# OSU-Bee-Lab/buzzdetect

Measured on AMD Instinct MI355X. Metric: yamnet_windows_per_s, higher is better.
Workload: dtype f32 (split-f16x3 MFMA products, f32 accumulate)

## Files before the change

buzzdetect_amd/csrc/bd_device.h:

```cpp
#pragma once

#include "bd_internal.h"

#include <mutex>
#include <type_traits>
#ifdef BD_KERNEL_TRACE
#include <cstdio>
#include <cstdlib>
#endif

namespace bd {

namespace {

typedef float f32x16 __attribute__((ext_vector_type(16)));
typedef float v2f __attribute__((ext_vector_type(2)));
typedef float v4f __attribute__((ext_vector_type(4)));
typedef unsigned v4u __attribute__((ext_vector_type(4)));
typedef unsigned u32x2 __attribute__((ext_vector_type(2)));
typedef _Float16 f16x2 __attribute__((ext_vector_type(2)));
typedef _Float16 f16x4 __attribute__((ext_vector_type(4)));
typedef _Float16 f16x8 __attribute__((ext_vector_type(8)));

constexpr float kF16Max = 65504.0f;
// ... 70 lines not shown
                                    }
                    }
    return true;
}
static_assert(tr_image_is_bijection(), "every (half, k, chunk) has its own 8 bytes of the slot, and they fill it");
static_assert(tr_image_writes_conflict_free(), "a lane group of the publication meets no bank twice");
static_assert(tr_image_reads_conflict_free(), "a lane half of the transposed read meets no bank twice");
__device__ __forceinline__ int tr_read_lane_off(int lane) {
    const int g = lane >> 4, q = (lane >> 2) & 3, p = lane & 3;
    return tr_image_off(0, tr_read_k(0, g >> 1, 0, q), tr_read_chunk(0, g & 1, p));
}
__host__ __device__ constexpr int tr_read_next(int off) { return (off ^ 16) + 4 * kTrRowBytes; }
constexpr bool tr_read_next_holds() {
    for (int lane = 0; lane < 64; ++lane) {
        const int g = lane >> 4, q = (lane >> 2) & 3, p = lane & 3;
        if (tr_read_next(tr_image_off(0, tr_read_k(0, g >> 1, 0, q), tr_read_chunk(0, g & 1, p))) !=
            tr_image_off(0, tr_read_k(0, g >> 1, 1, q), tr_read_chunk(0, g & 1, p)))
            return false;
        for (int s = 0; s < 2; ++s)
            for (int i = 0; i < 3; ++i)
                for (int r = 0; r < 2; ++r)
                    if (tr_image_off(0, tr_read_k(s, g >> 1, r, q), tr_read_chunk(i, g & 1, p)) !=
                        tr_image_off(0, tr_read_k(0, g >> 1, r, q), tr_read_chunk(0, g & 1, p)) + 16 * s * kTrRowBytes + 64 * i)
                        return false;
    }
    return true;
}
static_assert(tr_read_next_holds(), "the reader's immediates");
__device__ __forceinline__ f16x8 tr_read_frag(const char* p0, const char* p1) {
    typedef short s16x4 __attribute__((ext_vector_type(4)));
    typedef __attribute__((address_space(3))) s16x4* lds4;
    const s16x4 a = __builtin_amdgcn_ds_read_tr16_b64_v4i16((lds4)p0), b = __builtin_amdgcn_ds_read_tr16_b64_v4i16((lds4)p1);
    return __builtin_bit_cast(f16x8, __builtin_shufflevector(a, b, 0, 1, 2, 3, 4, 5, 6, 7));
}

__device__ __forceinline__ unsigned pw_lds_addr(const void* p) {
    return (unsigned)(unsigned long long)(__attribute__((address_space(3))) const void*)p;
}
template <int OFFSET>
__device__ __forceinline__ f16x8 pw_lds_frag(unsigned addr) {
    f16x8 v;
    asm volatile("ds_read_b128 %0, %1 offset:%2" : "=v"(v) : "v"(addr), "n"(OFFSET) : "memory");
    return v;
}
__device__ __forceinline__ void pw_lds_store64(unsigned addr, f16x4 v) {
    asm volatile("ds_write_b64 %0, %1" ::"v"(addr), "v"(v) : "memory");
}
__device__ __forceinline__ f16x8 pw_landed(f16x8 v) {
    asm volatile("" : "+v"(v));
    return v;
}
template <int N>
__device__ __forceinline__ void pw_lds_wait() {
    asm volatile("s_waitcnt lgkmcnt(%0)" ::"n"(N) : "memory");
}
template <int I, int E, typename F>
__device__ __forceinline__ void static_for_pw(F&& f) {
    if constexpr (I < E) {
        f(std::integral_constant<int, I>{});
        static_for_pw<I + 1, E>(f);
    }
}
template <int K16, int V, int R>
struct PwResSchedule {
    static constexpr int split_at(int q) {
        for (int j = 0; j < V; ++j)
// ... 60 lines not shown
```

buzzdetect_amd/csrc/bd_internal.h:

```cpp
#pragma once

#include <hip/hip_runtime.h>
#include <stdint.h>

#include <string>
#include <vector>

#include "../../include/buzzdetect_hip.h"

namespace bd {

constexpr int kMelNonZero = 461;

constexpr int kMelStart[BD_MEL_BANDS] = {
    5, 5, 6, 7, 9, 10, 11, 12, 13, 14, 16, 17, 18, 20, 21, 23, 25, 26, 28, 30, 32, 34, 36, 38, 40, 42, 44, 47, 49, 52, 54, 57,
    60, 63, 66, 69, 72, 76, 79, 83, 87, 90, 95, 99, 103, 108, 112, 117, 122, 127, 133, 138, 144, 150, 156, 162, 169, 176, 183,
    190, 198, 206, 214, 223};
constexpr int kMelLen[BD_MEL_BANDS] = {
    1, 2, 3, 3, 2, 2, 2, 2, 3, 3, 2, 3, 3, 3, 4, 3, 3, 4, 4, 4, 4, 4, 4, 4, 4, 5, 5, 5, 5, 5, 6, 6,
    6, 6, 6, 7, 7, 7, 8, 7, 8, 9, 8, 9, 9, 9, 10, 10, 11, 11, 11, 12, 12, 12, 13, 14, 14, 14, 15, 16, 16, 17, 17, 17};
constexpr int mel_offset(int band) {
    int o = 0;
    for (int m = 0; m < band; ++m) o += kMelLen[m];
    return o;
// ... 133 lines not shown
                  const SepLayer& L2, const SepLayer& L3, float* out, hipStream_t stream);

void launch_stem_reg(const float* logmel, int patch_step, const WindowMap& map, int w0, int windows, const float* c1_w,
                     const float* c1_b, const SepLayer& L2, const SepLayer& L3, float* out, hipStream_t stream);
void launch_stem_reg_planes(const float* logmel, int patch_step, const WindowMap& map, int w0, int windows, const float* c1_w,
                            const float* c1_b, const SepLayer& L2, const SepLayer& L3, float* out, hipStream_t stream);

void launch_stem_reg_f32(const float* logmel, int patch_step, const WindowMap& map, int w0, int windows, const float* c1_w,
                         const float* c1_b, const SepLayer& L2, const SepLayer& L3, float* out, hipStream_t stream);

bool launch_l4_reg_f32(const float* in, float* out, int windows, const SepLayer& L4, const SepLayer& L5, hipStream_t stream);

bool launch_separable_mid(const float* in, float* out, int windows, const SepLayer& L5, const SepLayer& L6, const SepLayer& L7,
                          hipStream_t stream);
constexpr int kDw7PlaneBytes = 8 * 2 * 24 * 32 * 2;
bool separable_mid_planes_supported(const SepLayer& L5, const SepLayer& L6, const SepLayer& L7);
bool launch_separable_mid_planes(const float* in, void* out, int windows, const SepLayer& L5, const SepLayer& L6, const SepLayer& L7,
                                 hipStream_t stream);

bool launch_separable_mid_f32(const float* in, float* out, int windows, const SepLayer& L5, const SepLayer& L6, const SepLayer& L7,
                              hipStream_t stream);

bool separable_chip_pw7_supported(const SepLayer& L7, const SepLayer* L, int nl, const SepLayer& next, int windows);
bool launch_separable_chip_pw7(const void* in, float* out, int windows, const SepLayer& L7, const SepLayer* L, int nl,
                               const SepLayer& next, hipStream_t stream);
int launch_separable_run_next_dw(const float* a, float* b, int windows, const SepLayer* L, int max_layers, hipStream_t stream,
                                 bool planes = false);

bool launch_separable_chip_f32(const float* in, float* out, int windows, const SepLayer* L, int nl, hipStream_t stream,
                               const SepLayer* next, bool dw0_done);

bool tail_supported(const SepLayer& L13, const SepLayer& L14);
bool launch_tail_pw13_dw14(const void* in, void* out, int windows, const SepLayer& L13, const SepLayer& L14, hipStream_t stream);
bool launch_tail_pw14_pool(const void* in, float* pooled, int windows, const SepLayer& L14, hipStream_t stream);
bool tail_f32_supported(const SepLayer& L13, const SepLayer& L14);
bool launch_tail_f32(const float* in, float* mid, float* pooled, int windows, const SepLayer& L13, const SepLayer& L14, hipStream_t stream,
                     int which);

struct DenseLayer {
    int k, n;
    int act;
    const float* wfrag;
    const float* bias;
};
size_t dense_packed_floats(int k, int n);
void dense_pack_weights(const float* kernel, int k, int n, float* dst);
void launch_dense(const float* A, int lda, int windows, const DenseLayer& L, float* C, int ldc, hipStream_t stream);
void launch_softmax_rows(const float* x, int ldx, float* y, int windows, int n, hipStream_t stream);

}

struct bd_headset_member;

namespace bd {

constexpr int kHeadSetRow = 2048;
constexpr int kHeadSetRegions = 3;
struct HeadSet {
    int members = 0, outputs = 0;
    std::vector<int> first, count;
    std::vector<int> last_act;
    char* dev = nullptr;
    struct Depth {
        const void* layers;
        const void* tiles;
        int n_tiles;
    };
// ... 33 lines not shown
```

buzzdetect_amd/csrc/cnn.hip:

```cpp
#include "bd_device.h"

namespace bd {

namespace {

constexpr int kC1Rows = 4;

__global__ __launch_bounds__(256) void conv1_kernel(const float* __restrict__ logmel, int patch_step,
                                                    const WindowMap map, int w0,
                                                    const float* __restrict__ w9x32,
                                                    const float* __restrict__ b32,
                                                    float* __restrict__ out) {
    const int tid = threadIdx.x;
    const int c4 = tid & 7;
    const int ow = tid >> 3;
    const int win = blockIdx.y;
    const float* patch = logmel + window_frame(map, w0 + win, patch_step) * BD_MEL_BANDS;

    float4 wt[9];
#pragma unroll
    for (int t = 0; t < 9; ++t) wt[t] = reinterpret_cast<const float4*>(w9x32 + t * 32)[c4];
    const float4 bias = reinterpret_cast<const float4*>(b32)[c4];

#pragma unroll
// ... 609 lines not shown
    __shared__ float s_part[4][BD_MAX_CLASSES];
    const int tid = threadIdx.x;
    const int lane = tid & 63;
    const int wave = tid >> 6;
    const size_t win = blockIdx.x;
    const float4* src = reinterpret_cast<const float4*>(act + win * POOL * BD_EMBEDDING_SIZE);
    float4 s = src[tid];
    if constexpr (POOL > 1) {
#pragma unroll
        for (int p = 1; p < POOL; ++p) {
            const float4 v = src[p * (BD_EMBEDDING_SIZE / 4) + tid];
            s.x += v.x;
            s.y += v.y;
            s.z += v.z;
            s.w += v.w;
        }
        s.x /= (float)POOL;
        s.y /= (float)POOL;
        s.z /= (float)POOL;
        s.w /= (float)POOL;
        if (emb) reinterpret_cast<float4*>(emb + win * BD_EMBEDDING_SIZE)[tid] = s;
    }
    if (!logits) return;

    for (int c0 = 0; c0 < n_classes; c0 += 16) {
        float4 w[16];
#pragma unroll
        for (int j = 0; j < 16; ++j) {
            const int c = c0 + j < n_classes ? c0 + j : n_classes - 1;
            w[j] = reinterpret_cast<const float4*>(head_wt + (size_t)c * BD_EMBEDDING_SIZE)[tid];
        }
        float p[16];
#pragma unroll
        for (int j = 0; j < 16; ++j) p[j] = fmaf(s.x, w[j].x, fmaf(s.y, w[j].y, fmaf(s.z, w[j].z, s.w * w[j].w)));
#pragma unroll
        for (int o = 32; o > 0; o >>= 1)
#pragma unroll
            for (int j = 0; j < 16; ++j) p[j] += __shfl_xor(p[j], o, 64);
#pragma unroll
        for (int j = 0; j < 16; ++j)
            if (lane == 0 && c0 + j < n_classes) s_part[wave][c0 + j] = p[j];
    }
    __syncthreads();
    if (tid < n_classes)
        logits[win * n_classes + tid] =
            ((s_part[0][tid] + s_part[1][tid]) + (s_part[2][tid] + s_part[3][tid])) + head_b[tid];
}

}

void launch_conv1(const float* logmel, int patch_step, const WindowMap& map, int w0, int windows, const float* w9x32,
                  const float* b32, float* out, hipStream_t stream) {
    if (windows <= 0) return;
    hipLaunchKernelGGL(conv1_kernel, dim3(48 / kC1Rows, windows), dim3(256), 0, stream, logmel, patch_step, map, w0,
                       w9x32, b32, out);
}

template <int STRIDE, int OWB>
static void launch_dw(const float* in, float* out, int windows, const SepLayer& L, hipStream_t stream) {
    const long long total = (long long)windows * L.h_out * (L.w_out / OWB) * (L.cin / 4);
    const long long blocks = (total + 255) / 256;
    const int grid = (int)(blocks < (1 << 20) ? blocks : (1 << 20));
    hipLaunchKernelGGL((depthwise_kernel<STRIDE, OWB>), dim3(grid), dim3(256), 0, stream, in, out, dw_w_of(L), dw_b_of(L),
                       windows, L.h_in, L.w_in, L.cin, L.h_out, L.w_out, L.amax);
}

void launch_scale_copy(const float* src, float* dst, int64_t n, float factor, hipStream_t stream) {
// ... 164 lines not shown
```

buzzdetect_amd/csrc/engine.hip:

```cpp
#include <cmath>
#include <cstdio>
#include <cstdlib>
#include <cstring>
#include <unistd.h>
#include <memory>
#include <string>
#include <type_traits>
#include <utility>
#include <vector>

#include "bd_internal.h"

#include "../../include/buzzdetect_anyrate.h"
#include "../../include/buzzdetect_head.h"
#include "../../include/buzzdetect_headset.h"
#include "../../include/buzzdetect_ensemble.h"

namespace {

thread_local std::string g_error;

int fail(int code, const std::string& msg) {
    g_error = msg;
    return code;
// ... 2 lines not shown
#define BD_HIP(expr)                                                                            \
    do {                                                                                        \
        hipError_t e_ = (expr);                                                                 \
        if (e_ != hipSuccess)                                                                   \
            return fail(BD_EHIP, std::string(#expr) + ": " + hipGetErrorString(e_));            \
    } while (0)

const int kLayerDefs[14][2] = {{2, 32},  {1, 64},  {2, 128}, {1, 128}, {2, 256}, {1, 256},  {2, 512},
                               {1, 512}, {1, 512}, {1, 512}, {1, 512}, {1, 512}, {2, 1024}, {1, 1024}};

constexpr int64_t kFloatsA = 98304;
constexpr int64_t kFloatsB = 49152;
constexpr int kDefaultGroup = 1024;
constexpr int kMaxGroup = 65536;
static_assert(kMaxGroup <= 1 << 17, "the tail launchers of pass_f16 / pass_f32 cover the largest pass");
static_assert(bd::kDw7PlaneBytes <= kFloatsA * 4, "the depthwise-7 planes of the middle run fit buffer a");

inline int64_t align_up(int64_t v, int64_t a) { return (v + a - 1) / a * a; }

struct Event2 {
    hipEvent_t ev;
    int slot;
};

}

struct bd_engine {
    int device = 0;
    int n_classes = 0;
    int group_windows = kDefaultGroup;
    int pointwise_mode = 1;
    unsigned* d_range_flag = nullptr;
    int stem = 3, separable = 1;
    float* d_pool = nullptr;
    bd::FeTables* d_tables = nullptr;
    std::vector<float> h_dw[13];
    std::vector<int> row_exp[13];
    size_t off_dw16[13] = {0}, off_pw_u[13] = {0};
    float act_max[13] = {0};
    int act_exp[13] = {0};
    unsigned* d_amax = nullptr;
    const float* conv1_w = nullptr;
    const float* conv1_b = nullptr;
    bd::SepLayer sep[13];
    const float* head_wt = nullptr;
    const float* head_b = nullptr;
    std::vector<bd::DenseLayer> stack;
    float* d_stack = nullptr;
    bd::HeadSet set;
    bd::Ensemble ens;
    struct Taps {
        int up, down, quality, half;
        float* dev;
        std::vector<float> host;
        bool has_plan;
        bd::FirPlanHost fir;
        hipStream_t upload_stream;
        hipEvent_t uploaded;
    };
    std::vector<Taps> taps;
    struct AnyTaps {
        bd::AnyratePlan plan;
        int quality;
        float* dev;
        std::vector<float> host;
        hipStream_t upload_stream;
// ... 345 lines not shown
            const int kq = cin / 16;
            for (int n = 0; n < cout; ++n)
                for (int k = 0; k < cin; ++k) {
                    const int lane = (n & 31) + 32 * ((k & 15) >> 3);
                    const size_t dst = (((size_t)(n >> 5) * kq + (k >> 4)) * 64 + lane) * 8 + (k & 7);
                    fhi[dst] = hi[(size_t)n * cin + k];
                    flo[dst] = lo[(size_t)n * cin + k];
                }
        }
        off_pw_ffrag[l] = 0;
        if (cin >= 128) {
            off_pw_ffrag[l] = reserve(nw);
            const float* wf = host.data() + off_pw_w[l];
            float* ff = host.data() + off_pw_ffrag[l];
            const int ks = cin / 8;
            for (int n = 0; n < cout; ++n)
                for (int k = 0; k < cin; ++k) {
                    const int lane = (n & 31) + 32 * ((k & 7) >> 2);
                    ff[(((size_t)(n >> 5) * ks + (k >> 3)) * 64 + lane) * 4 + (k & 3)] = wf[(size_t)n * cin + k];
                }
        }
        cin = cout;
    }
    if (p - w->embedder_blob != BD_EMBEDDER_BLOB_FLOATS) return fail(BD_EWEIGHTS, "internal: blob walk mismatch");
    size_t off_head_w = 0, off_head_b = 0;
    if (w->n_classes > 0) {
        off_head_w = reserve((size_t)w->n_classes * BD_EMBEDDING_SIZE);
        off_head_b = reserve(BD_MAX_CLASSES);
        for (int c = 0; c < w->n_classes; ++c)
            for (int k = 0; k < BD_EMBEDDING_SIZE; ++k)
                host[off_head_w + (size_t)c * BD_EMBEDDING_SIZE + k] = w->head_kernel[(size_t)k * w->n_classes + c];
        for (int c = 0; c < w->n_classes; ++c) host[off_head_b + c] = w->head_bias[c];
    }
    {
        bool finite = true;
        for (size_t i = off_conv1_w; i < off_conv1_b + 32; ++i) finite = finite && std::isfinite(host[i]);
        int c = kLayerDefs[0][1];
        for (int l = 0; l < 13; ++l) {
            const int co = kLayerDefs[l + 1][1];
            for (size_t i = 0; i < 9 * (size_t)c; ++i) finite = finite && std::isfinite(host[off_dw_w[l] + i]);
            for (int i = 0; i < c; ++i) finite = finite && std::isfinite(host[off_dw_b[l] + i]);
            for (size_t i = 0; i < (size_t)c * co; ++i) finite = finite && std::isfinite(host[off_pw_w[l] + i]);
            for (int i = 0; i < co; ++i) finite = finite && std::isfinite(host[off_pw_b[l] + i]);
            c = co;
        }
        if (!finite) return fail(BD_EWEIGHTS, "bd_create: non-finite value after BatchNorm folding");
    }

    bd::FeTables tables;
    int rc = build_tables(w->mel, &tables);
    if (rc < 0) return rc;

    bd_engine* e = new bd_engine();
    e->device = device;
    e->n_classes = w->n_classes;
    hipError_t err = hipMalloc(&e->d_pool, host.size() * sizeof(float));
    if (err == hipSuccess) err = hipMalloc(&e->d_tables, sizeof(bd::FeTables));
    if (err == hipSuccess) err = hipMalloc(&e->d_range_flag, 256);
    if (err == hipSuccess) err = hipMemset(e->d_range_flag, 0, 256);
    if (err == hipSuccess) err = hipMalloc(&e->d_amax, 64);
    if (err == hipSuccess) err = hipMemset(e->d_amax, 0, 64);
    if (err == hipSuccess) err = hipMemcpy(e->d_pool, host.data(), host.size() * sizeof(float), hipMemcpyHostToDevice);
    if (err == hipSuccess) err = hipMemcpy(e->d_tables, &tables, sizeof(tables), hipMemcpyHostToDevice);
    if (err != hipSuccess) {
        if (e->d_pool) (void)hipFree(e->d_pool);
        if (e->d_tables) (void)hipFree(e->d_tables);
        if (e->d_range_flag) (void)hipFree(e->d_range_flag);
        if (e->d_amax) (void)hipFree(e->d_amax);
        delete e;
        return fail(BD_EHIP, std::string("bd_create: ") + hipGetErrorString(err));
    }
    e->conv1_w = e->d_pool + off_conv1_w;
    e->conv1_b = e->d_pool + off_conv1_b;
    int h = 48, wd = 32;
    cin = kLayerDefs[0][1];
    for (int l = 0; l < 13; ++l) {
        bd::SepLayer& L = e->sep[l];
        L.cin = cin;
        L.cout = kLayerDefs[l + 1][1];
        L.stride = kLayerDefs[l + 1][0];
        L.h_in = h;
        L.w_in = wd;
        L.h_out = (h + L.stride - 1) / L.stride;
        L.w_out = (wd + L.stride - 1) / L.stride;
        L.dw_w = e->d_pool + off_dw_w[l];
        L.dw_b = e->d_pool + off_dw_b[l];
        L.pw_wt = e->d_pool + off_pw_w[l];
        L.pw_b = e->d_pool + off_pw_b[l];
        L.pw_variant = 0;
        L.pw_whi = e->d_pool + off_pw_hi[l];
        L.pw_wlo = e->d_pool + off_pw_lo[l];
        L.pw_fhi = e->d_pool + off_pw_fhi[l];
        L.pw_flo = e->d_pool + off_pw_flo[l];
        L.pw_ffrag = off_pw_ffrag[l] ? e->d_pool + off_pw_ffrag[l] : nullptr;
        L.pw_variant16 = 0;
        L.pw_mode = e->pointwise_mode;
        L.range_flag = e->d_range_flag;
        L.dw_w16 = e->d_pool + off_dw16[l];
        L.dw_b16 = L.dw_w16 + 9 * (size_t)cin;
        L.pw_u = e->d_pool + off_pw_u[l];
        L.act_exp = 0;
        L.amax = nullptr;
        e->off_dw16[l] = off_dw16[l];
        e->off_pw_u[l] = off_pw_u[l];
        e->row_exp[l] = row_exps[l];
// ... 450 lines not shown
        stem(g, bd::launch_stem_reg_planes);
        if (!g.launch(7, [&] { return bd::launch_l4_window_planes(g.a, sep[1], sep[2], sep[3], g.b, g.gw, g.stream); }))
            return fail(BD_EHIP, "l4_window_kernel declined the planes of the stem");
    } else {
        if (e->stem != 0) {
            stem(g, e->stem == 3 ? bd::launch_stem_reg : bd::launch_stem4);
        } else {
            conv1(g);
            walk_layers(g, 0, false, 4);
        }
        if (e->separable == 0) return walk_layers(g, 2, false, -1);
        if (!g.launch(7, [&] { return bd::launch_separable_fused_next_dw(g.a, g.b, g.gw, sep[2], sep[3], g.stream); }))
            return walk_layers(g, 2, false, -1);
    }
    const bool planes = bd::tail_supported(sep[11], sep[12]);
    if (e->separable == 1 && planes && bd::separable_mid_planes_supported(sep[3], sep[4], sep[5]) &&
        bd::separable_chip_pw7_supported(sep[5], &sep[6], 5, sep[11], g.gw)) {
        if (!g.launch(13, [&] { return bd::launch_separable_mid_planes(g.b, g.a, g.gw, sep[3], sep[4], sep[5], g.stream); }))
            return fail(BD_EHIP, "sep_mid_kernel declined the depthwise-7 planes");
        if (!g.launch(23, [&] { return bd::launch_separable_chip_pw7(g.a, g.b, g.gw, sep[5], &sep[6], 5, sep[11], g.stream); }))
            return fail(BD_EHIP, "sep_chip_kernel declined the planes of the middle run");
    } else {
        if (!(e->separable == 1 &&
              g.launch(13, [&] { return bd::launch_separable_mid(g.b, g.a, g.gw, sep[3], sep[4], sep[5], g.stream); }))) {
            pointwise(g, 3);
            if (!g.launch(11, [&] { return bd::launch_separable_fused_next_dw(g.a, g.b, g.gw, sep[4], sep[5], g.stream); }))
                return walk_layers(g, 4, false, -1);
            pointwise(g, 5);
        }
        if (!g.launch(23, [&] { return bd::launch_separable_run_next_dw(g.a, g.b, g.gw, &sep[6], 7, g.stream, planes); }))
            return walk_layers(g, 6, false, -1);
        if (!planes) return walk_layers(g, 11, true, -1);
    }
    float* const pooled = g.emb ? g.emb : g.b;
    if (!g.launch(25, [&] { return bd::launch_tail_pw13_dw14(g.b, g.a, g.gw, sep[11], sep[12], g.stream); }) ||
        !g.launch(27, [&] { return bd::launch_tail_pw14_pool(g.a, pooled, g.gw, sep[12], g.stream); }))
        return fail(BD_EHIP, "septail.hip declined the planes of the on-chip run");
    return head(g, pooled);
}

int pass_f32(Group& g) {
    const bd_engine* e = g.e;
    const bd::SepLayer* sep = g.sep;
    stem(g, bd::launch_stem_reg_f32);
    if (e->separable == 0) return walk_layers(g, 2, false, -1);
    if (!g.launch(7, [&] { return bd::launch_l4_reg_f32(g.a, g.b, g.gw, sep[2], sep[3], g.stream); }))
        return walk_layers(g, 2, false, -1);
    bool dw8_done = false;
    if (!(e->separable == 1 &&
          g.launch(13, [&] { return bd::launch_separable_mid_f32(g.b, g.a, g.gw, sep[3], sep[4], sep[5], g.stream); }))) {
        for (int l = 3; l < 6; ++l) {
            if (!g.launch(3 + 2 * l, [&] { return bd::launch_pointwise_next_dw_f32(g.b, g.a, g.gw, sep[l], sep[l + 1], g.stream); }))
                return walk_layers(g, l, true, -1);
            std::swap(g.a, g.b);
        }
        dw8_done = true;
    }
    if (!g.launch(23, [&] {
            return dw8_done ? bd::launch_separable_chip_f32(g.b, g.a, g.gw, &sep[6], 5, g.stream, &sep[11], true)
                            : bd::launch_separable_chip_f32(g.a, g.b, g.gw, &sep[6], 5, g.stream, &sep[11], false);
        }))
        return walk_layers(g, 6, dw8_done, -1);
    if (dw8_done) std::swap(g.a, g.b);
    if (!bd::tail_f32_supported(sep[11], sep[12])) return walk_layers(g, 11, true, -1);
    float* const pooled = g.emb ? g.emb : g.b;
    if (!g.launch(25, [&] { return bd::launch_tail_f32(g.b, g.a, pooled, g.gw, sep[11], sep[12], g.stream, 0); }) ||
        !g.launch(27, [&] { return bd::launch_tail_f32(g.b, g.a, pooled, g.gw, sep[11], sep[12], g.stream, 1); }))
        return fail(BD_EHIP, "septail.hip declined the exact-f32 tail");
    return head(g, pooled);
// ... 288 lines not shown
        if (act_exp[l] < -60 || act_exp[l] > 60) return fail(BD_EINVAL, "bd_set_activation_exponents: exponent outside -60..60");
    for (int l = 0; l < 13; ++l) h->act_exp[l] = act_exp[l];
    return apply_scales(h);
}

int bd_stage_tap(bd_handle h, const float* pcm_dev, int64_t n_samples, int32_t hop_samples, int32_t patch_step,
                 void* workspace_dev, int64_t workspace_bytes, int32_t stage, int32_t windows, float* out_dev,
                 void* stream) {
    if (!out_dev) return fail(BD_EINVAL, "bd_stage_tap: null output");
    if (stage < 0 || stage >= BD_NUM_STAGES) return fail(BD_EINVAL, "bd_stage_tap: stage out of range");
    return run_packed(h, pcm_dev, &n_samples, 1, hop_samples, patch_step, workspace_dev, workspace_bytes, nullptr,
                      nullptr, stage, windows, out_dev, (hipStream_t)stream);
}

int bd_debug_pointwise(const float* a_dev, const float* wt_dev, const float* bias_dev, float* c_dev, int64_t m,
                       int32_t n, int32_t k, int32_t variant, void* stream) {
    if (!a_dev || !wt_dev || !bias_dev || !c_dev || m < 0) return fail(BD_EINVAL, "bd_debug_pointwise: bad argument");
    if (bd::launch_pointwise_variant(a_dev, wt_dev, bias_dev, c_dev, m, n, k, variant, (hipStream_t)stream) != 0)
        return fail(BD_EINVAL, "bd_debug_pointwise: shape/variant not supported (K % 32, N % tile)");
    BD_HIP(hipGetLastError());
    return BD_OK;
}

int bd_set_pointwise_variant(bd_handle h, int32_t layer, int32_t variant) {
    if (!h || layer < 2 || layer > 14) return fail(BD_EINVAL, "bd_set_pointwise_variant: layer must be 2..14");
    if (h->sep[layer - 2].pw_mode != 0) h->sep[layer - 2].pw_variant16 = variant;
    else h->sep[layer - 2].pw_variant = variant;
    return BD_OK;
}

int bd_set_fusion(bd_handle h, int32_t stem, int32_t separable) {
    if (!h) return fail(BD_EINVAL, "null handle");
    if (stem != 0 && stem != 3 && stem != 5) return fail(BD_EINVAL, "bd_set_fusion: stem must be 0, 3 or 5");
    if (separable != 0 && separable != 1 && separable != 10)
        return fail(BD_EINVAL, "bd_set_fusion: separable must be 0, 1 or 10");
    h->stem = stem;
    h->separable = separable;
    return BD_OK;
}

int bd_range_flag(bd_handle h, int32_t* flag_host, int32_t reset, void* stream) {
    if (!h || !flag_host) return fail(BD_EINVAL, "bd_range_flag: null argument");
    BD_HIP(hipSetDevice(h->device));
    unsigned v = 0;
    BD_HIP(hipMemcpyAsync(&v, h->d_range_flag, sizeof(v), hipMemcpyDeviceToHost, (hipStream_t)stream));
    BD_HIP(hipStreamSynchronize((hipStream_t)stream));
    if (reset && v) BD_HIP(hipMemsetAsync(h->d_range_flag, 0, sizeof(v), (hipStream_t)stream));
    *flag_host = (int32_t)v;
    return BD_OK;
}

int bd_range_flag_copy(bd_handle h, int32_t* dst, int32_t reset, void* stream) {
    if (!h || !dst) return fail(BD_EINVAL, "bd_range_flag_copy: null argument");
    BD_HIP(hipSetDevice(h->device));
    BD_HIP(hipMemcpyAsync(dst, h->d_range_flag, sizeof(int32_t), hipMemcpyDefault, (hipStream_t)stream));
    if (reset) BD_HIP(hipMemsetAsync(h->d_range_flag, 0, sizeof(int32_t), (hipStream_t)stream));
    return BD_OK;
}

int bd_set_pointwise_mode(bd_handle h, int32_t mode) {
    if (!h || mode < 0 || mode > 2)
        return fail(BD_EINVAL, "bd_set_pointwise_mode: mode must be 0 (f32), 1 (split f16) or 2 (plain f16)");
    h->pointwise_mode = mode;
    for (auto& L : h->sep) L.pw_mode = mode;
    return BD_OK;
}

int bd_debug_pointwise_f16x3(const float* a_dev, const void* whi_dev, const void* wlo_dev, const float* unscale_dev,
                             const float* bias_dev, float* c_dev, int64_t m, int32_t n, int32_t k, int32_t variant,
                             void* stream) {
// ... 259 lines not shown
```

buzzdetect_amd/csrc/septail.hip:

```cpp
#include "bd_device.h"

#include <type_traits>

namespace bd {

namespace {

constexpr int kTailN = 1024;
constexpr int kTailPlane = 96 * 128;
constexpr int kTailStage = 2 * kTailPlane;
constexpr int kTailRing = 4;
constexpr int kTailLds = kTailRing * kTailStage;

struct TailArgs {
    const _Float16 *ahi, *alo;
    const _Float16 *bhi, *blo;
    const float *pu, *pb;
    const float* taps;
    _Float16 *ohi, *olo;
    float* pooled;
};

#define TAIL_RSRC(P, BYTES) __builtin_amdgcn_make_buffer_rsrc(const_cast<void*>(static_cast<const void*>(P)), 0, (BYTES), 0x00020000)

template <int K, int EPI, bool PLAIN, bool TRACE = false>
__global__ __launch_bounds__(256) __attribute__((amdgpu_waves_per_eu(1, 1))) void tail_gemm_kernel(const TailArgs a, int M, int windows,
                                                                                                 unsigned* __restrict__ range_flag,
                                                                                                 unsigned long long* __restrict__ dbg = nullptr) {
    extern __shared__ __attribute__((aligned(16))) char sm[];
    int tsn = 0;
#define TAIL_TS()                                                                                         \
    if constexpr (TRACE) {                                                                                \
        if ((blockIdx.x == 0 || blockIdx.x == 101) && threadIdx.x == 0 && tsn < 32)                       \
            dbg[(blockIdx.x ? 32 : 0) + tsn] = __builtin_amdgcn_s_memtime();                              \
        ++tsn;                                                                                            \
    }
    if constexpr (TRACE) {
        if (blockIdx.x == 0 && threadIdx.x == 0) dbg[30] = wall_clock64();
    }
    TAIL_TS()
    constexpr int N = kTailN, NST = K / 64, KQ = K / 16;
    constexpr int NB = PLAIN ? 2 : 4;
    constexpr int ND = PLAIN ? 3 : 6;
    const int tid = threadIdx.x, lane = tid & 63;
    const int wc = __builtin_amdgcn_readfirstlane(tid >> 6);
    const int frow = lane & 31, fh = lane >> 5;
    const int xcd = blockIdx.x & 7, kx = blockIdx.x >> 3;
    const int rt = 4 * (kx >> 1) + (xcd >> 1);
    const int m0 = rt * 96;
    if (m0 >= M) return;
    const int n0 = (2 * (xcd & 1) + (kx & 1)) * 256;
    const int x_cnt = M - m0 < 96 ? M - m0 : 96;

    const __amdgpu_buffer_rsrc_t ahr = TAIL_RSRC(a.ahi, (unsigned)M * K * 2), alr = TAIL_RSRC(a.alo, (unsigned)M * K * 2);
    unsigned dvo[3];
#pragma unroll
    for (int t = 0; t < 3; ++t) {
        const int L = (3 * wc + t) * 64 + lane;
// ... 5 lines not shown
    }
    auto dma1 = [&](int s, int t, bool lo) {
        char* const base = sm + (s % kTailRing) * kTailStage + 3 * wc * 1024 + t * 1024;
        if (lo) __builtin_amdgcn_raw_ptr_buffer_load_lds(alr, (__attribute__((address_space(3))) void*)(base + kTailPlane), 16, dvo[t], s * 128, 0, 0);
        else __builtin_amdgcn_raw_ptr_buffer_load_lds(ahr, (__attribute__((address_space(3))) void*)base, 16, dvo[t], s * 128, 0, 0);
    };
    auto dma = [&](int s) {
#pragma unroll
        for (int t = 0; t < 3; ++t) {
            dma1(s, t, false);
            if constexpr (!PLAIN) dma1(s, t, true);
        }
    };
    unsigned aro[2][4];
#pragma unroll
    for (int s = 0; s < 4; ++s) {
        aro[0][s] = frow * 128 + (((2 * s + fh) ^ ((frow >> 1) & 7)) << 4);
        aro[1][s] = aro[0][s] + 2 * kTailStage;
    }
    const __amdgpu_buffer_rsrc_t bhr = TAIL_RSRC(a.bhi, N * K * 2), blr = TAIL_RSRC(a.blo, N * K * 2);
    const int sb0 = (n0 / 32 + 2 * wc) * KQ * 1024;
    unsigned bvo[2];
#pragma unroll
    for (int j = 0; j < 2; ++j) bvo[j] = (frow >> 4) * (KQ * 1024) + ((((2 * frow + j) & 31) + 32 * fh) << 4);
    f16x8 bh[4][2], bl[4][2];
    const int ch0 = n0 + 64 * wc + 2 * frow;
    const v2f u2 = *reinterpret_cast<const v2f*>(a.pu + ch0), b2 = *reinterpret_cast<const v2f*>(a.pb + ch0);
    v2f wt2[9], shift2;
    if constexpr (EPI == 0) {
#pragma unroll
        for (int t = 0; t < 9; ++t) wt2[t] = *reinterpret_cast<const v2f*>(a.taps + t * N + ch0);
        shift2 = *reinterpret_cast<const v2f*>(a.taps + 9 * N + ch0);
    }

    dma(0);
    asm volatile("" ::: "memory");
#pragma unroll
    for (int s = 1; s < kTailRing - 1; ++s) dma(s);
#define TAIL_BLOAD(S, J, Q)                                                                               \
    {                                                                                                     \
        bh[S][J] = __builtin_bit_cast(f16x8, __builtin_amdgcn_raw_buffer_load_b128(bhr, bvo[J], sb0 + (Q) * 1024, 0)); \
        if constexpr (!PLAIN)                                                                             \
            bl[S][J] = __builtin_bit_cast(f16x8, __builtin_amdgcn_raw_buffer_load_b128(blr, bvo[J], sb0 + (Q) * 1024, 0)); \
    }
#pragma unroll
    for (int s = 0; s < 4; ++s) {
        TAIL_BLOAD(s, 0, s)
        TAIL_BLOAD(s, 1, s)
    }
    f32x16 acc[3][2];
    {
        float zero;
        asm volatile("v_mov_b32 %0, 0" : "=v"(zero));
#pragma unroll
        for (int i = 0; i < 3; ++i)
#pragma unroll
            for (int j = 0; j < 2; ++j)
#pragma unroll
                for (int r = 0; r < 16; ++r) acc[i][j][r] = zero;
    }
    asm volatile("s_waitcnt vmcnt(%0)" ::"n"(4 * NB + (kTailRing - 2) * ND) : "memory");
    __builtin_amdgcn_s_barrier();
    asm volatile("" ::: "memory");
    TAIL_TS()

    f16x8 ah[2][3], al[2][3];
// ... 32 lines not shown
                }
            } else if (k < NAL + 2) {
                if (lb) TAIL_BLOAD(br, k - NAL, g + 3)
            } else if ((g & 3) == 2 && (g >> 2) + kTailRing - 1 < NST) {
                if constexpr (PLAIN) {
                    if (k == NAL + 2) dma((g >> 2) + kTailRing - 1);
                } else if (k < NAL + 2 + ND) {
                    dma1((g >> 2) + kTailRing - 1, (k - NAL - 2) >> 1, (k - NAL - 2) & 1);
                }
            }
            __builtin_amdgcn_sched_barrier(0);
        }
        if ((g & 3) == 1 && (g >> 2) + 1 < NST) {
            asm volatile("s_waitcnt vmcnt(%0)" ::"n"(2 * NB) : "memory");
            __builtin_amdgcn_s_barrier();
            asm volatile("" ::: "memory");
            __builtin_amdgcn_sched_barrier(0);
        }
        if constexpr (TRACE) {
            if ((g & 3) == 3) { TAIL_TS() }
        }
    }
#undef TAIL_ALOAD
#undef TAIL_BLOAD

    v2f yv[48];
#pragma unroll
    for (int n = 0; n < 48; ++n) {
        const v2f c2 = {acc[n >> 4][0][n & 15], acc[n >> 4][1][n & 15]};
        const v2f y = __builtin_elementwise_fma(c2, u2, b2);
        yv[n] = v2f{fmaxf(y.x, 0.0f), fmaxf(y.y, 0.0f)};
    }
    if constexpr (EPI == 1) {
        const __amdgpu_buffer_rsrc_t pr = TAIL_RSRC(a.pooled, (unsigned)windows * N * 4);
        const unsigned po = (unsigned)((m0 / 6 + 8 * fh) * N + ch0) * 4;
#pragma unroll
        for (int w = 0; w < 8; ++w) {
            float sx = yv[6 * w].x, sy = yv[6 * w].y;
#pragma unroll
            for (int p = 1; p < 6; ++p) {
                sx += yv[6 * w + p].x;
                sy += yv[6 * w + p].y;
            }
            const float six = 6.0f;
            sx /= six;
            sy /= six;
            __builtin_amdgcn_raw_buffer_store_b64(u32x2{__builtin_bit_cast(unsigned, sx), __builtin_bit_cast(unsigned, sy)}, pr, po, w * N * 4, 0);
        }
    } else {
        float rmax = 0.0f;
        const __amdgpu_buffer_rsrc_t ohr = TAIL_RSRC(a.ohi + (size_t)m0 * N, (unsigned)x_cnt * N * 2);
        const __amdgpu_buffer_rsrc_t olr = TAIL_RSRC(a.olo + (size_t)m0 * N, (unsigned)x_cnt * N * 2);
        const unsigned oo = (unsigned)(48 * fh * N + ch0) * 2;
#pragma unroll
        for (int w = 0; w < 8; ++w)
#pragma unroll
            for (int oy = 0; oy < 3; ++oy)
#pragma unroll
                for (int ox = 0; ox < 2; ++ox) {
                    v2f s2 = shift2;
#pragma unroll
                    for (int kh = 0; kh < 3; ++kh)
#pragma unroll
                        for (int kw = 0; kw < 3; ++kw) {
                            const int iy = oy + kh - 1, ix = ox + kw - 1;
                            if (iy < 0 || iy >= 3 || ix < 0 || ix >= 2) continue;
                            s2 = __builtin_elementwise_fma(yv[6 * w + 2 * iy + ix], wt2[kh * 3 + kw], s2);
                        }
                    const float ox_ = fmaxf(s2.x, 0.0f), oy_ = fmaxf(s2.y, 0.0f);
                    unsigned hi2, lo2;
                    asm volatile("v_cvt_pk_f16_f32 %0, %3, %4\n\t"
                                 "v_fma_mixlo_f16 %1, %0, -1.0, %3 op_sel:[0,0,0] op_sel_hi:[1,0,0]\n\t"
                                 "v_fma_mixhi_f16 %1, %0, -1.0, %4 op_sel:[1,0,0] op_sel_hi:[1,0,0]\n\t"
                                 "v_max3_f32 %2, %2, |%3|, |%4|"
                                 : "=&v"(hi2), "=&v"(lo2), "+v"(rmax)
                                 : "v"(ox_), "v"(oy_));
                    const int so = (6 * w + 2 * oy + ox) * N * 2;
                    __builtin_amdgcn_raw_buffer_store_b32(hi2, ohr, oo, so, 0);
                    if constexpr (!PLAIN) __builtin_amdgcn_raw_buffer_store_b32(lo2, olr, oo, so, 0);
                }
// ... 158 lines not shown
    } else {
        const __amdgpu_buffer_rsrc_t orr = TAIL_RSRC(a.out + (size_t)m0 * N, (unsigned)x_cnt * N * 4);
        const unsigned oo = (unsigned)(48 * fh * N + ch0) * 4;
#pragma unroll
        for (int w = 0; w < 8; ++w)
#pragma unroll
            for (int oy = 0; oy < 3; ++oy)
#pragma unroll
                for (int ox = 0; ox < 2; ++ox) {
                    v2f s2 = shift2;
#pragma unroll
                    for (int kh = 0; kh < 3; ++kh)
#pragma unroll
                        for (int kw = 0; kw < 3; ++kw) {
                            const int iy = oy + kh - 1, ix = ox + kw - 1;
                            if (iy < 0 || iy >= 3 || ix < 0 || ix >= 2) continue;
                            s2 = __builtin_elementwise_fma(yv[6 * w + 2 * iy + ix], wt2[kh * 3 + kw], s2);
                        }
                    const float ox_ = fmaxf(s2.x, 0.0f), oy_ = fmaxf(s2.y, 0.0f);
                    __builtin_amdgcn_raw_buffer_store_b64(u32x2{__builtin_bit_cast(unsigned, ox_), __builtin_bit_cast(unsigned, oy_)}, orr, oo,
                                                          (6 * w + 2 * oy + ox) * N * 4, 0);
                }
    }
}

template <int K, int EPI>
void launch_tail_f32(const TailArgsF32& a, int windows, hipStream_t stream) {
    allow_dynamic_lds<&tail_gemm_f32_kernel<K, EPI>>(kTailLds);
    const int M = windows * 6;
    const int nrt4 = ((M + 95) / 96 + 3) / 4 * 4;
    hipLaunchKernelGGL((tail_gemm_f32_kernel<K, EPI>), dim3(4 * nrt4), dim3(256), kTailLds, stream, a, M, windows);
}

template <int K, int EPI, bool PLAIN>
void launch_tail(const TailArgs& a, int windows, unsigned* range_flag, hipStream_t stream) {
    allow_dynamic_lds<&tail_gemm_kernel<K, EPI, PLAIN>>(kTailLds);
    const int M = windows * 6;
    const int nrt4 = ((M + 95) / 96 + 3) / 4 * 4;
#ifdef BD_KERNEL_TRACE
    bool printed = false;
    if (const unsigned long long* h = traced_launch(
            '9', &tail_gemm_kernel<K, EPI, PLAIN, true>, kTailLds, stream, 32, 101, &printed,
            [&](unsigned long long* dbg) {
                hipLaunchKernelGGL((tail_gemm_kernel<K, EPI, PLAIN, true>), dim3(4 * nrt4), dim3(256), kTailLds, stream, a, M, windows, range_flag, dbg);
            },
            "tail, workgroup %d, K = %d: cycles between stamps (prologue | one per stage | epilogue | stores land):", K)) {
        if (printed) fprintf(stderr, "[trace] ... workgroup 0 lived %llu ticks of the 100 MHz clock\n", h[31] - h[30]);
        return;
    }
#endif
    hipLaunchKernelGGL((tail_gemm_kernel<K, EPI, PLAIN>), dim3(4 * nrt4), dim3(256), kTailLds, stream, a, M, windows, range_flag);
}

}

bool tail_supported(const SepLayer& L13, const SepLayer& L14) {
    if (L13.cin != 512 || L13.cout != 1024 || L13.h_out != 3 || L13.w_out != 2 || L14.cin != 1024 || L14.cout != 1024 || L14.stride != 1 ||
        L14.h_out != 3 || L14.w_out != 2)
        return false;
    return L13.pw_mode != 0 && L14.pw_mode == L13.pw_mode && dw_b_of(L14) == dw_w_of(L14) + 9 * 1024;
}

bool launch_tail_pw13_dw14(const void* in, void* out, int windows, const SepLayer& L13, const SepLayer& L14, hipStream_t stream) {
    if (windows <= 0 || windows > (1 << 18) || in == out || !tail_supported(L13, L14)) return false;
    const size_t rows = (size_t)windows * 6;
    TailArgs a{};
    a.ahi = static_cast<const _Float16*>(in);
    a.alo = a.ahi + rows * 512;
    a.bhi = static_cast<const _Float16*>(L13.pw_fhi);
    a.blo = static_cast<const _Float16*>(L13.pw_flo);
    a.pu = L13.pw_u;
    a.pb = L13.pw_b;
    a.taps = dw_w_of(L14);
    a.ohi = static_cast<_Float16*>(out);
    a.olo = a.ohi + rows * 1024;
    if (L13.pw_mode == 2) launch_tail<512, 0, true>(a, windows, L14.range_flag, stream);
    else launch_tail<512, 0, false>(a, windows, L14.range_flag, stream);
    return true;
}

bool launch_tail_pw14_pool(const void* in, float* pooled, int windows, const SepLayer& L14, hipStream_t stream) {
    if (windows <= 0 || windows > (1 << 18)) return false;
    if (L14.cin != 1024 || L14.cout != 1024 || L14.h_out != 3 || L14.w_out != 2 || L14.pw_mode == 0) return false;
    const size_t rows = (size_t)windows * 6;
    TailArgs a{};
    a.ahi = static_cast<const _Float16*>(in);
    a.alo = a.ahi + rows * 1024;
    a.bhi = static_cast<const _Float16*>(L14.pw_fhi);
    a.blo = static_cast<const _Float16*>(L14.pw_flo);
    a.pu = L14.pw_u;
    a.pb = L14.pw_b;
    a.pooled = pooled;
    if (L14.pw_mode == 2) launch_tail<1024, 1, true>(a, windows, nullptr, stream);
    else launch_tail<1024, 1, false>(a, windows, nullptr, stream);
    return true;
}

bool tail_f32_supported(const SepLayer& L13, const SepLayer& L14) {
    return L13.cin == 512 && L13.cout == 1024 && L13.h_out == 3 && L13.w_out == 2 && L14.cin == 1024 && L14.cout == 1024 && L14.stride == 1 &&
           L14.h_out == 3 && L14.w_out == 2 && L13.pw_ffrag && L14.pw_ffrag;
}
bool launch_tail_f32(const float* in, float* mid, float* pooled, int windows, const SepLayer& L13, const SepLayer& L14, hipStream_t stream,
                     int which) {
    if (windows <= 0 || windows > (1 << 17) || !tail_f32_supported(L13, L14)) return false;
    TailArgsF32 a{};
    if (which == 0) {
        a.a = in;
        a.bfrag = L13.pw_ffrag;
        a.pb = L13.pw_b;
        a.taps = L14.dw_w;
        a.tshift = L14.dw_b;
        a.out = mid;
        launch_tail_f32<512, 0>(a, windows, stream);
    } else {
        a.a = mid;
        a.bfrag = L14.pw_ffrag;
        a.pb = L14.pw_b;
        a.pooled = pooled;
        launch_tail_f32<1024, 1>(a, windows, stream);
    }
    return true;
}

}
```

Measured before the change: 2.056 million.

## Fuse classifier head into pw14 pool kernel with ticketed cross-block reduction

Computes the classifier head's partial dot products inside the final pointwise+pool tail kernel. Each column-block writes per-window partial logits through LDS and a DPP row reduction, and the last arriving block per row tile (atomic ticket) combines the partials and adds the bias. This removes the separate head kernel launch and the round trip of pooled embeddings through memory. In exchange it adds head-weight register pressure, extra barriers and atomics in the tail epilogue, and it is gated off when profiling, headsets or stacks are active.

```diff
diff --git a/buzzdetect_amd/csrc/bd_device.h b/buzzdetect_amd/csrc/bd_device.h
--- a/buzzdetect_amd/csrc/bd_device.h
+++ b/buzzdetect_amd/csrc/bd_device.h
@@ -126,6 +126,18 @@
     typedef __attribute__((address_space(3))) s16x4* lds4;
     const s16x4 a = __builtin_amdgcn_ds_read_tr16_b64_v4i16((lds4)p0), b = __builtin_amdgcn_ds_read_tr16_b64_v4i16((lds4)p1);
     return __builtin_bit_cast(f16x8, __builtin_shufflevector(a, b, 0, 1, 2, 3, 4, 5, 6, 7));
+}
+
+__device__ __forceinline__ float dense_quad(float sx, float sy, float sz, float sw, float wx, float wy, float wz, float ww) {
+    return fmaf(sx, wx, fmaf(sy, wy, fmaf(sz, wz, sw * ww)));
+}
+__device__ __forceinline__ float lane_xor1(float v) {
+    return __builtin_bit_cast(float, __builtin_amdgcn_update_dpp(0, __builtin_bit_cast(int, v), 0xB1, 0xF, 0xF, false));
+}
+template <int N>
+__device__ __forceinline__ float row_ror(float v) {
+    static_assert(N >= 1 && N <= 15, "row_ror:1 .. row_ror:15");
+    return __builtin_bit_cast(float, __builtin_amdgcn_update_dpp(0, __builtin_bit_cast(int, v), 0x120 + N, 0xF, 0xF, false));
 }
 
 __device__ __forceinline__ unsigned pw_lds_addr(const void* p) {
diff --git a/buzzdetect_amd/csrc/bd_internal.h b/buzzdetect_amd/csrc/bd_internal.h
--- a/buzzdetect_amd/csrc/bd_internal.h
+++ b/buzzdetect_amd/csrc/bd_internal.h
@@ -189,7 +189,20 @@
 
 bool tail_supported(const SepLayer& L13, const SepLayer& L14);
 bool launch_tail_pw13_dw14(const void* in, void* out, int windows, const SepLayer& L13, const SepLayer& L14, hipStream_t stream);
-bool launch_tail_pw14_pool(const void* in, float* pooled, int windows, const SepLayer& L14, hipStream_t stream);
+struct TailHead {
+    const float* head_wt;
+    const float* head_b;
+    int n_classes;
+    float* partials;
+    unsigned* tickets;
+    float* logits;
+};
+constexpr int kTailHeadWindows = 16;
+inline size_t tail_head_partial_floats(int windows) {
+    return (size_t)((windows + kTailHeadWindows - 1) / kTailHeadWindows) * kTailHeadWindows * 4 * BD_MAX_CLASSES;
+}
+bool launch_tail_pw14_pool(const void* in, float* pooled, int windows, const SepLayer& L14, hipStream_t stream,
+                           const TailHead* head = nullptr);
 bool tail_f32_supported(const SepLayer& L13, const SepLayer& L14);
 bool launch_tail_f32(const float* in, float* mid, float* pooled, int windows, const SepLayer& L13, const SepLayer& L14, hipStream_t stream,
                      int which);
diff --git a/buzzdetect_amd/csrc/cnn.hip b/buzzdetect_amd/csrc/cnn.hip
--- a/buzzdetect_amd/csrc/cnn.hip
+++ b/buzzdetect_amd/csrc/cnn.hip
@@ -665,7 +665,7 @@
         }
         float p[16];
 #pragma unroll
-        for (int j = 0; j < 16; ++j) p[j] = fmaf(s.x, w[j].x, fmaf(s.y, w[j].y, fmaf(s.z, w[j].z, s.w * w[j].w)));
+        for (int j = 0; j < 16; ++j) p[j] = dense_quad(s.x, s.y, s.z, s.w, w[j].x, w[j].y, w[j].z, w[j].w);
 #pragma unroll
         for (int o = 32; o > 0; o >>= 1)
 #pragma unroll
diff --git a/buzzdetect_amd/csrc/engine.hip b/buzzdetect_amd/csrc/engine.hip
--- a/buzzdetect_amd/csrc/engine.hip
+++ b/buzzdetect_amd/csrc/engine.hip
@@ -58,6 +58,8 @@
     int pointwise_mode = 1;
     unsigned* d_range_flag = nullptr;
     int stem = 3, separable = 1;
+    bool head_launch = false;
+    unsigned* head_tickets = nullptr;
     float* d_pool = nullptr;
     bd::FeTables* d_tables = nullptr;
     std::vector<float> h_dw[13];
@@ -469,6 +471,7 @@
                 host[off_head_w + (size_t)c * BD_EMBEDDING_SIZE + k] = w->head_kernel[(size_t)k * w->n_classes + c];
         for (int c = 0; c < w->n_classes; ++c) host[off_head_b + c] = w->head_bias[c];
     }
+    const size_t off_tickets = reserve(kMaxGroup / bd::kTailHeadWindows);
     {
         bool finite = true;
         for (size_t i = off_conv1_w; i < off_conv1_b + 32; ++i) finite = finite && std::isfinite(host[i]);
@@ -508,6 +511,7 @@
         return fail(BD_EHIP, std::string("bd_create: ") + hipGetErrorString(err));
     }
     e->conv1_w = e->d_pool + off_conv1_w;
+    e->head_tickets = reinterpret_cast<unsigned*>(e->d_pool + off_tickets);
     e->conv1_b = e->d_pool + off_conv1_b;
     int h = 48, wd = 32;
     cin = kLayerDefs[0][1];
@@ -1024,9 +1028,18 @@
             return walk_layers(g, 6, false, -1);
         if (!planes) return walk_layers(g, 11, true, -1);
     }
+    if (!g.launch(25, [&] { return bd::launch_tail_pw13_dw14(g.b, g.a, g.gw, sep[11], sep[12], g.stream); }))
+        return fail(BD_EHIP, "septail.hip declined the planes of the on-chip run");
+    if (g.logits && e->separable == 1 && !e->head_launch && !e->profiling && !e->set.members && e->stack.empty() && e->head_wt &&
+        e->n_classes > 0) {
+        static_assert(BD_EMBEDDING_SIZE + bd::kTailHeadWindows * 4 * BD_MAX_CLASSES <= kFloatsB, "the pooled row and a row tile's partial sums fit buffer b even for one window");
+        const bd::TailHead hd{e->head_wt, e->head_b, e->n_classes, g.b + (size_t)g.gw * BD_EMBEDDING_SIZE, e->head_tickets, g.logits};
+        if (!g.launch(27, [&] { return bd::launch_tail_pw14_pool(g.a, g.emb, g.gw, sep[12], g.stream, &hd); }))
+            return fail(BD_EHIP, "septail.hip declined the planes of the on-chip run");
+        return BD_OK;
+    }
     float* const pooled = g.emb ? g.emb : g.b;
-    if (!g.launch(25, [&] { return bd::launch_tail_pw13_dw14(g.b, g.a, g.gw, sep[11], sep[12], g.stream); }) ||
-        !g.launch(27, [&] { return bd::launch_tail_pw14_pool(g.a, pooled, g.gw, sep[12], g.stream); }))
+    if (!g.launch(27, [&] { return bd::launch_tail_pw14_pool(g.a, pooled, g.gw, sep[12], g.stream); }))
         return fail(BD_EHIP, "septail.hip declined the planes of the on-chip run");
     return head(g, pooled);
 }
@@ -1381,10 +1394,11 @@
 int bd_set_fusion(bd_handle h, int32_t stem, int32_t separable) {
     if (!h) return fail(BD_EINVAL, "null handle");
     if (stem != 0 && stem != 3 && stem != 5) return fail(BD_EINVAL, "bd_set_fusion: stem must be 0, 3 or 5");
-    if (separable != 0 && separable != 1 && separable != 10)
-        return fail(BD_EINVAL, "bd_set_fusion: separable must be 0, 1 or 10");
+    if (separable != 0 && separable != 1 && separable != 10 && separable != 13)
+        return fail(BD_EINVAL, "bd_set_fusion: separable must be 0, 1, 10 or 13");
     h->stem = stem;
-    h->separable = separable;
+    h->separable = separable == 13 ? 1 : separable;
+    h->head_launch = separable == 13;
     return BD_OK;
 }
 
diff --git a/buzzdetect_amd/csrc/septail.hip b/buzzdetect_amd/csrc/septail.hip
--- a/buzzdetect_amd/csrc/septail.hip
+++ b/buzzdetect_amd/csrc/septail.hip
@@ -19,11 +19,16 @@
     const float* taps;
     _Float16 *ohi, *olo;
     float* pooled;
+    TailHead head;
 };
 
+constexpr int kHeadTile = 16 * 4 * 16 * 64;
+static_assert(kHeadTile + 16 <= kTailLds, "the head's tile and its ticket word fit the A ring");
+__device__ __forceinline__ int head_tile_off(int win, int wave, int l, int g) { return ((win * 4 + wave) * 16 + l) * 64 + ((g ^ (l >> 2)) << 4); }
+
 #define TAIL_RSRC(P, BYTES) __builtin_amdgcn_make_buffer_rsrc(const_cast<void*>(static_cast<const void*>(P)), 0, (BYTES), 0x00020000)
 
-template <int K, int EPI, bool PLAIN, bool TRACE = false>
+template <int K, int EPI, bool PLAIN, bool TRACE = false, bool HEAD = false>
 __global__ __launch_bounds__(256) __attribute__((amdgpu_waves_per_eu(1, 1))) void tail_gemm_kernel(const TailArgs a, int M, int windows,
                                                                                                  unsigned* __restrict__ range_flag,
                                                                                                  unsigned long long* __restrict__ dbg = nullptr) {
@@ -95,6 +100,13 @@
         for (int t = 0; t < 9; ++t) wt2[t] = *reinterpret_cast<const v2f*>(a.taps + t * N + ch0);
         shift2 = *reinterpret_cast<const v2f*>(a.taps + 9 * N + ch0);
     }
+    static_assert(!HEAD || EPI == 1, "the head follows the pool");
+    v4f hw[16];
+    if constexpr (HEAD) {
+#pragma unroll
+        for (int j = 0; j < 16; ++j)
+            hw[j] = *reinterpret_cast<const v4f*>(a.head.head_wt + (size_t)(j < a.head.n_classes ? j : a.head.n_classes - 1) * N + (ch0 & ~3));
+    }
 
     dma(0);
     asm volatile("" ::: "memory");
@@ -193,8 +205,7 @@
         yv[n] = v2f{fmaxf(y.x, 0.0f), fmaxf(y.y, 0.0f)};
     }
     if constexpr (EPI == 1) {
-        const __amdgpu_buffer_rsrc_t pr = TAIL_RSRC(a.pooled, (unsigned)windows * N * 4);
-        const unsigned po = (unsigned)((m0 / 6 + 8 * fh) * N + ch0) * 4;
+        float px[8], py[8];
 #pragma unroll
         for (int w = 0; w < 8; ++w) {
             float sx = yv[6 * w].x, sy = yv[6 * w].y;
@@ -204,9 +215,104 @@
                 sy += yv[6 * w + p].y;
             }
             const float six = 6.0f;
-            sx /= six;
-            sy /= six;
-            __builtin_amdgcn_raw_buffer_store_b64(u32x2{__builtin_bit_cast(unsigned, sx), __builtin_bit_cast(unsigned, sy)}, pr, po, w * N * 4, 0);
+            px[w] = sx / six;
+            py[w] = sy / six;
+        }
+        if (!HEAD || a.pooled) {
+            const __amdgpu_buffer_rsrc_t pr = TAIL_RSRC(a.pooled, (unsigned)windows * N * 4);
+            const unsigned po = (unsigned)((m0 / 6 + 8 * fh) * N + ch0) * 4;
+#pragma unroll
+            for (int w = 0; w < 8; ++w)
+                __builtin_amdgcn_raw_buffer_store_b64(u32x2{__builtin_bit_cast(unsigned, px[w]), __builtin_bit_cast(unsigned, py[w])}, pr, po, w * N * 4, 0);
+        }
+        if constexpr (HEAD) {
+            TAIL_TS()
+            const TailHead& hd = a.head;
+            const int nc = hd.n_classes;
+            const bool odd = frow & 1;
+            const int l = frow >> 1, wt0 = 8 * fh + 4 * (frow & 1);
+            v4f s4[4];
+#pragma unroll
+            for (int i = 0; i < 4; ++i) {
+                const float rx = lane_xor1(odd ? px[i] : px[4 + i]), ry = lane_xor1(odd ? py[i] : py[4 + i]);
+                s4[i] = odd ? v4f{rx, ry, px[4 + i], py[4 + i]} : v4f{px[i], py[i], rx, ry};
+            }
+            const int rw = tid >> 4, rl = tid & 15;
+            const int prow = (rt * kTailHeadWindows + rw) * 4 + n0 / 256;
+            const __amdgpu_buffer_rsrc_t hpr = TAIL_RSRC(hd.partials, (unsigned)((windows + 15) / 16) * (16 * 4 * BD_MAX_CLASSES * 4));
+            for (int c0 = 0; c0 < nc; c0 += 16) {
+                const int ng = ((nc - c0 < 16 ? nc - c0 : 16) + 3) >> 2;
+                if (c0) {
+#pragma unroll
+                    for (int j = 0; j < 16; ++j)
+                        hw[j] = *reinterpret_cast<const v4f*>(hd.head_wt + (size_t)(c0 + j < nc ? c0 + j : nc - 1) * N + (ch0 & ~3));
+                }
+                __syncthreads();
+#pragma unroll
+                for (int g = 0; g < 4; ++g) {
+                    if (g < ng) {
+#pragma unroll
+                        for (int i = 0; i < 4; ++i) {
+                            v4f p;
+#pragma unroll
+                            for (int j = 0; j < 4; ++j)
+                                p[j] = dense_quad(s4[i].x, s4[i].y, s4[i].z, s4[i].w, hw[4 * g + j].x, hw[4 * g + j].y, hw[4 * g + j].z, hw[4 * g + j].w);
+                            *reinterpret_cast<v4f*>(sm + head_tile_off(wt0 + i, wc, l, g)) = p;
+                        }
+                    }
+                }
+                __syncthreads();
+                v4f t[4];
+#pragma unroll
+                for (int g = 0; g < 4; ++g) {
+                    if (g < ng) {
+                        const v4f q0 = *reinterpret_cast<const v4f*>(sm + head_tile_off(rw, 0, rl, g)), q1 = *reinterpret_cast<const v4f*>(sm + head_tile_off(rw, 1, rl, g));
+                        const v4f q2 = *reinterpret_cast<const v4f*>(sm + head_tile_off(rw, 2, rl, g)), q3 = *reinterpret_cast<const v4f*>(sm + head_tile_off(rw, 3, rl, g));
+                        t[g] = (q0 + q2) + (q1 + q3);
+#pragma unroll
+                        for (int j = 0; j < 4; ++j) {
+                            t[g][j] += row_ror<8>(t[g][j]);
+                            t[g][j] += row_ror<4>(t[g][j]);
+                            t[g][j] += row_ror<2>(t[g][j]);
+                            t[g][j] += row_ror<1>(t[g][j]);
+                        }
+                    } else {
+                        t[g] = v4f{0.0f, 0.0f, 0.0f, 0.0f};
+                    }
+                }
+                if (rl < ng) {
+                    const v4f o = rl == 0 ? t[0] : rl == 1 ? t[1] : rl == 2 ? t[2] : t[3];
+                    __builtin_amdgcn_raw_buffer_store_b128(__builtin_bit_cast(v4u, o), hpr, (unsigned)(prow * BD_MAX_CLASSES + c0 + 4 * rl) * 4, 0, 16);
+                }
+            }
+            TAIL_TS()
+            unsigned* const told = reinterpret_cast<unsigned*>(sm + kHeadTile);
+            asm volatile("s_waitcnt vmcnt(0)" ::: "memory");
+            __syncthreads();
+            if (tid == 0) *told = __hip_atomic_fetch_add(hd.tickets + rt, 1u, __ATOMIC_RELAXED, __HIP_MEMORY_SCOPE_AGENT);
+            __syncthreads();
+            if (*told != 3u) {
+                if constexpr (TRACE) {
+                    if (blockIdx.x == 0 && threadIdx.x == 0) dbg[31] = wall_clock64();
+                }
+                return;
+            }
+            TAIL_TS()
+            if (wc == 0) {
+                __builtin_amdgcn_fence(__ATOMIC_ACQUIRE, "agent");
+                asm volatile("s_waitcnt vmcnt(0)" ::: "memory");
+            }
+            __syncthreads();
+            const int win = rt * kTailHeadWindows + rw;
+            const float* const pw = hd.partials + (size_t)win * 4 * BD_MAX_CLASSES;
+            for (int c = rl; c < nc; c += 16) {
+                const float s0 = __hip_atomic_load(pw + c, __ATOMIC_RELAXED, __HIP_MEMORY_SCOPE_AGENT);
+                const float s1 = __hip_atomic_load(pw + BD_MAX_CLASSES + c, __ATOMIC_RELAXED, __HIP_MEMORY_SCOPE_AGENT);
+                const float s2 = __hip_atomic_load(pw + 2 * BD_MAX_CLASSES + c, __ATOMIC_RELAXED, __HIP_MEMORY_SCOPE_AGENT);
+                const float s3 = __hip_atomic_load(pw + 3 * BD_MAX_CLASSES + c, __ATOMIC_RELAXED, __HIP_MEMORY_SCOPE_AGENT);
+                if (win < windows) hd.logits[(size_t)win * nc + c] = ((s0 + s1) + (s2 + s3)) + hd.head_b[c];
+            }
+            if (tid == 0) __hip_atomic_store(hd.tickets + rt, 0u, __ATOMIC_RELAXED, __HIP_MEMORY_SCOPE_AGENT);
         }
     } else {
         float rmax = 0.0f;
@@ -431,24 +537,27 @@
     hipLaunchKernelGGL((tail_gemm_f32_kernel<K, EPI>), dim3(4 * nrt4), dim3(256), kTailLds, stream, a, M, windows);
 }
 
-template <int K, int EPI, bool PLAIN>
+template <int K, int EPI, bool PLAIN, bool HEAD = false>
 void launch_tail(const TailArgs& a, int windows, unsigned* range_flag, hipStream_t stream) {
-    allow_dynamic_lds<&tail_gemm_kernel<K, EPI, PLAIN>>(kTailLds);
+    allow_dynamic_lds<&tail_gemm_kernel<K, EPI, PLAIN, false, HEAD>>(kTailLds);
     const int M = windows * 6;
     const int nrt4 = ((M + 95) / 96 + 3) / 4 * 4;
 #ifdef BD_KERNEL_TRACE
     bool printed = false;
     if (const unsigned long long* h = traced_launch(
-            '9', &tail_gemm_kernel<K, EPI, PLAIN, true>, kTailLds, stream, 32, 101, &printed,
+            '9', &tail_gemm_kernel<K, EPI, PLAIN, true, HEAD>, kTailLds, stream, 32, 101, &printed,
             [&](unsigned long long* dbg) {
-                hipLaunchKernelGGL((tail_gemm_kernel<K, EPI, PLAIN, true>), dim3(4 * nrt4), dim3(256), kTailLds, stream, a, M, windows, range_flag, dbg);
+                hipLaunchKernelGGL((tail_gemm_kernel<K, EPI, PLAIN, true, HEAD>), dim3(4 * nrt4), dim3(256), kTailLds, stream, a, M, windows, range_flag, dbg);
             },
-            "tail, workgroup %d, K = %d: cycles between stamps (prologue | one per stage | epilogue | stores land):", K)) {
+            HEAD ? "tail + head, workgroup %d, K = %d: cycles between stamps (prologue | one per stage | pool | head partials | ticket | last arriver: "
+                   "combine | stores land):"
+                 : "tail, workgroup %d, K = %d: cycles between stamps (prologue | one per stage | epilogue | stores land):",
+            K)) {
         if (printed) fprintf(stderr, "[trace] ... workgroup 0 lived %llu ticks of the 100 MHz clock\n", h[31] - h[30]);
         return;
     }
 #endif
-    hipLaunchKernelGGL((tail_gemm_kernel<K, EPI, PLAIN>), dim3(4 * nrt4), dim3(256), kTailLds, stream, a, M, windows, range_flag);
+    hipLaunchKernelGGL((tail_gemm_kernel<K, EPI, PLAIN, false, HEAD>), dim3(4 * nrt4), dim3(256), kTailLds, stream, a, M, windows, range_flag);
 }
 
 }
@@ -478,8 +587,12 @@
     return true;
 }
 
-bool launch_tail_pw14_pool(const void* in, float* pooled, int windows, const SepLayer& L14, hipStream_t stream) {
+bool launch_tail_pw14_pool(const void* in, float* pooled, int windows, const SepLayer& L14, hipStream_t stream, const TailHead* head) {
     if (windows <= 0 || windows > (1 << 18)) return false;
+    if (!head && !pooled) return false;
+    if (head && (windows > (1 << 16) || head->n_classes < 1 || head->n_classes > BD_MAX_CLASSES || !head->head_wt || !head->head_b || !head->partials ||
+                 !head->tickets || !head->logits || (reinterpret_cast<uintptr_t>(head->partials) & 15u)))
+        return false;
     if (L14.cin != 1024 || L14.cout != 1024 || L14.h_out != 3 || L14.w_out != 2 || L14.pw_mode == 0) return false;
     const size_t rows = (size_t)windows * 6;
     TailArgs a{};
@@ -490,6 +603,12 @@
     a.pu = L14.pw_u;
     a.pb = L14.pw_b;
     a.pooled = pooled;
+    if (head) {
+        a.head = *head;
+        if (L14.pw_mode == 2) launch_tail<1024, 1, true, true>(a, windows, nullptr, stream);
+        else launch_tail<1024, 1, false, true>(a, windows, nullptr, stream);
+        return true;
+    }
     if (L14.pw_mode == 2) launch_tail<1024, 1, true>(a, windows, nullptr, stream);
     else launch_tail<1024, 1, false>(a, windows, nullptr, stream);
     return true;
```

Result: no change. 2.071 million, median of 6 (+0.7%).
